# patngnw/NewsRecommendation

Measured on AMD Instinct MI355X. Metric: train impressions/sec @ batch 512, NRMS, higher is better.
Workload: dtype bf16; 1 GPU; NRMS train step (fwd+bwd+Adam), MIND-small shapes: title_len=30, history=50, npratio=4, 300-d word table; per_gpu_batch=512, global_batch=512, vocab_rows=30000, freeze_embedding=False, compact_history=False, dense_batch=False, feed=resident, deterministic=False, optimizer=flat bucket + HIP fused Adam, parallelism=dp1

## Files before the change

newsrecommendation_amd/csrc/nr_api.hip:

```cpp
#include <stdarg.h>
#include <stdio.h>
#include <stdlib.h>
#include <string.h>

#include "nr_gemm.h"

int nr_launch_attn(bool bwd, int dtype, const void* qkv, const float* mask, void* y, const void* dy, void* dqkv, int n, int L,
                   int heads, int d_head, const DropCfg& drop, hipStream_t stream, const uint32_t* tmask = nullptr,
                   const float* bias = nullptr, const int32_t* seq_list = nullptr, const int32_t* seq_count = nullptr,
                   const int32_t* needed = nullptr);
bool nr_attn_pad_ok(int dtype, int L, int d_head, const void* p0, const void* p1);
bool nr_attn_rowsub_ok(int dtype, int L, int d_head, int heads);
bool nr_attn_compact_ok(int dtype, int L, int d_head, int heads);
int nr_launch_attn_bwd_compact(const void* qkv, const float* mask, const void* dy, void* dqkv, int n, int L, int heads, int d_head,
                               const DropCfg& drop, hipStream_t stream, const uint32_t* tmask, const float* bias, const int32_t* seq_list,
                               const int32_t* seq_count, const int32_t* pos, void* dump, float* db, const int32_t* nzf);
int nr_launch_attn_gather_fwd(const void* proj_table, const int32_t* ids, const float* mask, void* y, int n, int L, int heads,
                              int d_head, const DropCfg& drop, hipStream_t stream);
int nr_launch_pool_core_fwd(int dtype, const void* x, const void* e, const float* w2, const float* b2, const float* mask,
                            float* alpha, float* out, int ld_out, int n, int L, int N, int q, hipStream_t s,
                            const int32_t* needed = nullptr);
int nr_launch_pool_core_bwd(int dtype, const void* x, const void* e, const float* w2, const float* alpha, const float* g,
                            int ld_g, void* dpre, float* partial, float* dw2, float* db2, int n, int L, int N, int q,
                            hipStream_t s, const int32_t* seq_nz = nullptr);
// ... 963 lines not shown
  return nr_launch_pool_core_fwd(d->dtype, d->x, e, d->w2, d->b2, d->mask, alpha, out, ld_out, d->n, d->L, d->N, d->q, s, d->seq_needed);
}

int nr_additive_pool_bwd(const nr_pool_desc* d, const void* e, const float* alpha, const float* g, int ld_g, const void* w1_t,
                         int ldw1t, void* dpre, float* partial, float* dw1, float* db1, float* dw2, float* db2, void* dx,
                         nr_stream_t stream) {
  int rc = pool_check(d);
  if (rc) return rc;
  if (d->n == 0) return NR_OK;
  NR_CHECK_ARG(e && alpha && g && dpre && partial && dw1 && db1 && dw2 && db2, "additive_pool_bwd: null operand");
  NR_DEVICE_GUARD(stream, dpre);
  NR_CHECK_ARG(d->partial_bytes >= pool_ws_elems(d->n, d->L, d->q, d->N, d->dtype) * sizeof(float),
               "additive_pool_bwd: partial holds %zu bytes, nr_pool_workspace_bytes() asks for %zu", d->partial_bytes,
               pool_ws_elems(d->n, d->L, d->q, d->N, d->dtype) * sizeof(float));
  float* tn_scratch = partial + pool_ws_ints(d->n, d->L, d->q);
  const size_t tn_floats = pool_tn_floats(d->n, d->L, d->q, d->N, d->dtype);
  hipStream_t s = (hipStream_t)stream;
  const int M = d->n * d->L;
  DetScope det(s);
  det.add(dw1, (size_t)d->q * d->N);
  det.add(db1, (size_t)d->q);
  det.add(dw2, (size_t)d->q);
  det.add(db2, 1);
  if ((rc = det.begin(true, true))) return rc;
  int32_t* ws = nullptr;
  if (pool_has_flags(d)) {
    ws = reinterpret_cast<int32_t*>(partial + pool_ws_used(d->n, d->q));
    if ((rc = nr_launch_row_flags_f32(g, ld_g, d->N, d->n, ws, s))) return rc;
  }
  const int32_t* zero_flags = ws != nullptr ? ws : d->seq_needed;
  if (ws != nullptr && dx != nullptr && w1_t != nullptr && !det.on() && nr_pool_fused_bwd_ok(d->dtype, d->n, d->L, d->N, d->q, ldw1t) && ld_g % 4 == 0 &&
      ((((uintptr_t)d->x) | ((uintptr_t)e) | ((uintptr_t)w1_t) | ((uintptr_t)dpre) | ((uintptr_t)dx) | ((uintptr_t)g)) & 15) == 0 && d->N % 8 == 0) {
    int rows = 0;
    if ((rc = nr_launch_pool_fused_bwd(d->x, d->N, e, d->q, alpha, g, ld_g, d->w2, w1_t, ldw1t, dpre, d->q, dx, d->N, partial,
                                       nr_pool_partial_rows(d->n), ws, d->n, d->L, d->N, d->q, s, &rows, d->dx_far_unwritten)))
      return rc;
    if ((rc = nr_launch_colsum_split(partial, rows, d->q + 1, d->q + 1, dw2, d->q, db2, s))) return rc;
    if ((rc = nr_launch_live_slabs(ws, d->n, d->L, s))) return rc;
    return gemm_tn_live_slabs(ws, d->n, dpre, d->q, d->x, d->N, dw1, d->N, db1, M, d->q, d->N, d->q, d->N, s, 0, tn_scratch, tn_floats);
  }
  if ((rc = nr_launch_pool_core_bwd(d->dtype, d->x, e, d->w2, alpha, g, ld_g, dpre, partial, dw2, db2, d->n, d->L, d->N, d->q, s, zero_flags)))
    return rc;
  RowSrc X = dense_rows(d->x, d->N, d->N);
  if (ws != nullptr) {
    if ((rc = nr_launch_live_slabs(ws, d->n, d->L, s))) return rc;
    if ((rc = gemm_tn_live_slabs(ws, d->n, dpre, d->q, d->x, d->N, dw1, d->N, db1, M, d->q, d->N, d->q, d->N, s, 0, tn_scratch, tn_floats))) return rc;
  } else if ((rc = nr_launch_gemm_tn(d->dtype, dpre, d->q, X, dw1, d->N, db1, M, d->q, d->N, d->q, d->N, s))) {
    return rc;
  }
  if (dx != nullptr) {
    NR_CHECK_ARG(w1_t != nullptr && ldw1t >= d->q, "additive_pool_bwd: w1_t [N, >=q] needed for dx");
    RowSrc P = dense_rows(dpre, d->q, d->q);
    EpiArgs ep = store_epi(dx, d->N, d->dtype, nullptr, 0);
    ep.rowscale = alpha; ep.G = g; ep.ldg = ld_g; ep.L = d->L;
    ep.seq_nz = zero_flags;
    rc = nr_launch_gemm_nt(d->dtype, P, w1_t, ldw1t, M, d->N, d->q, EPI_POOLBWD, ep, s);
  }
  return rc;
}

static int linear_rows(const nr_linear_desc* d, RowSrc* out) {
  NR_CHECK_ARG(d != nullptr, "linear: null descriptor");
  NR_CHECK_ARG(dtype_ok(d->dtype), "linear: bad dtype %d", d->dtype);
  const int ch = nr_chunk(d->dtype);
  NR_CHECK_ARG(d->M >= 0 && d->K >= 1 && d->N >= 1, "linear: bad shape M=%d K=%d N=%d", d->M, d->K, d->N);
  NR_CHECK_ARG(d->ldx >= round_up(d->K, ch) && d->ldw >= round_up(d->K, ch), "linear: ldx=%d / ldw=%d must cover K=%d rounded up to %d",
               d->ldx, d->ldw, d->K, ch);
  NR_CHECK_ARG(d->M == 0 || (d->x && d->w), "linear: null operand");
  RowSrc s = dense_rows(d->x, d->ldx, d->K);
  if (d->src_kind == NR_SRC_GATHER) {
    NR_CHECK_ARG(d->ids != nullptr && d->ids_stride >= 1, "linear: gather source without ids");
// ... 54 lines not shown
```

newsrecommendation_amd/csrc/nr_attn_mfma.hip:

```cpp
#include <stdlib.h>
#include <type_traits>

#include "nr_common.h"

namespace {

constexpr int AW = 4;

template <typename T> struct AT;
template <> struct AT<bf16_t> { static constexpr int SW = 40; };
template <> struct AT<float> { static constexpr int SW = 36; };

struct AttnMArgs {
  const void* qkv;
  const float* mask;
  void* y;
  const void* dy;
  void* dqkv;
  int n, L, heads, d, N;
  int vec;
  float scale;
  DropCfg drop;
  const int32_t* seq_list;
  const int32_t* seq_count;
// ... 1057 lines not shown
          const bf16_t* src = img0 + re * ops + pc.q4(t);
          *reinterpret_cast<bf16x4*>(base + off) = *reinterpret_cast<const bf16x4*>(src);
          *reinterpret_cast<bf16x4*>(base + off + N) = *reinterpret_cast<const bf16x4*>(src + 32 * ops);
          *reinterpret_cast<bf16x4*>(base + off + 2 * N) = *reinterpret_cast<const bf16x4*>(src + 64 * ops);
        }
      } else if (FULL) {
        panel_store_all<PT>(img0, ops, op, N3, pc);
        panel_store_all<PT>(img0 + 32 * ops, ops, op + N, N3, pc);
        panel_store_all<PT>(img0 + 64 * ops, ops, op + 2 * N, N3, pc);
      } else {
        panel_store<PT>(img0, ops, op, N3, pc, hcount);
        panel_store<PT>(img0 + 32 * ops, ops, op + N, N3, pc, hcount);
        panel_store<PT>(img0 + 64 * ops, ops, op + 2 * N, N3, pc, hcount);
      }
    } else {
      bf16_t* op = dqkv + row0 * N3 + (active ? head : 0) * d;
      acc_t_to_global<false>(dq, op, N3, Ls, d, lane, nodrop, 0, 0);
      acc_t_to_global<false>(dk, op + N, N3, Ls, d, lane, nodrop, 0, 0);
      acc_t_to_global<false>(dv, op + 2 * N, N3, Ls, d, lane, nodrop, 0, 0);
    }
    __syncthreads();
    put(pf);
    __syncthreads();
  }
  if (CPT) {
    for (int i = tid; i < hgroups * AW * 3 * DBS; i += AW * 64) {
      const int c = i % DBS, mat = (i / DBS) % 3, head = i / (3 * DBS);
      if (c < d && head < heads) atomicAdd(a.db + mat * N + head * d + c, sDb[i]);
    }
  }
}


__device__ __forceinline__ int clampL(int L, int rb) { return min(32, max(0, L - 32 * rb)); }

template <bool GATHER, int LC = 0, int DC = 0, int HC = 0>
__global__ __launch_bounds__(AW * 64) __attribute__((amdgpu_waves_per_eu(2, 2))) void fwd64_kernel(AttnMArgs a) {
  extern __shared__ __attribute__((aligned(16))) char smem[];
  const int lane = threadIdx.x & 63, wid = __builtin_amdgcn_readfirstlane(threadIdx.x >> 6);
  bf16_t* base = reinterpret_cast<bf16_t*>(smem) + (size_t)wid * 7 * IMG;
  bf16_t *sQ = base, *sK = base + 2 * IMG, *sV = base + 4 * IMG, *sO = base + 6 * IMG;
  float* sMask = reinterpret_cast<float*>(reinterpret_cast<bf16_t*>(smem) + (size_t)AW * 7 * IMG) + wid * 64;
  const bf16_t* qkv = reinterpret_cast<const bf16_t*>(a.qkv);
  bf16_t* y = reinterpret_cast<bf16_t*>(a.y);
  const int L = LC ? LC : a.L, d = DC ? DC : a.d, heads = HC ? HC : a.heads, N = heads * d, h2 = lane >> 5;
  DropCfg nodrop;
  nodrop.key = 0; nodrop.thresh = 0; nodrop.scale = 1.f;
  const int hgroups = (heads + AW - 1) / AW;
  Slice t[2][3];
  int idr[2] = {0, 0};
  int sh_n = 0, ln_n = L, sh_c = 0, ln_c = L;
  bool gen_n = false, gen_c = false;
  auto load_ids = [&](long sb) {
    if (GATHER) {
      const size_t row0 = (size_t)sb * L;
      sh_n = 0; ln_n = L; gen_n = false;
      if (a.mask != nullptr) {
        const float mv = lane < L ? a.mask[row0 + lane] : 0.f;
        const unsigned long long bal = __ballot(mv != 0.f);
        if (bal == 0) {
          sh_n = L; ln_n = 0;
        } else {
          const int s0 = __builtin_ctzll(bal), hi = 64 - __builtin_clzll(bal);
          if (__popcll(bal) == hi - s0) { sh_n = s0; ln_n = hi - s0; } else gen_n = true;
        }
      }
// ... 26 lines not shown
#pragma unroll
        for (int w = 0; w < 3; ++w) slice_load(t[rb][w], src + (size_t)32 * rb * 3 * N + w * N, 3 * N, Lr, d, lane);
      }
    }
  };
  long sb = blockIdx.x;
  if (sb >= a.n) return;
  load_ids(sb);
  load(sb, 0);
  for (; sb < a.n; sb += gridDim.x)
    for (int hgi = 0; hgi < hgroups; ++hgi) {
      const int hraw = hgi * AW + wid;
      const bool active = hraw < heads;
      if (GATHER && hgi == 0) { sh_c = sh_n; ln_c = ln_n; gen_c = gen_n; }
      const int Lc = GATHER ? ln_c : L;
      const bool two = Lc > 32;
      const int head = active ? hraw : 0, Lw = active ? Lc : 0;
      const size_t row0 = (size_t)sb * L;
#pragma unroll
      for (int rb = 0; rb < 2; ++rb) {
        const int Lr = clampL(Lw, rb);
        slice_put<false>(t[rb][0], Lr, d, sQ + rb * IMG, lane, nodrop, 0, 0);
        slice_put<false>(t[rb][1], Lr, d, sK + rb * IMG, lane, nodrop, 0, 0);
        slice_put<false>(t[rb][2], Lr, d, sV + rb * IMG, lane, nodrop, 0, 0);
      }
      sMask[lane] = (lane < Lw) ? ((a.mask && (!GATHER || gen_c)) ? a.mask[row0 + lane] : 1.f) : 0.f;
      if (GATHER && Lc < L) {
        const int hcols = min(AW, heads - hgi * AW) * d, ppr = hcols >> 2, nz = (L - Lc) * ppr;
        for (int u = threadIdx.x; u < nz; u += AW * 64) {
          const int i = u / ppr, c = (u - i * ppr) * 4, row = i < sh_c ? i : i + Lc;
          *reinterpret_cast<bf16x4*>(y + (row0 + row) * N + hgi * AW * d + c) = (bf16x4){(bf16_t)0.f, (bf16_t)0.f, (bf16_t)0.f, (bf16_t)0.f};
        }
      }
      __syncthreads();
      float mk0[16], mk1[16];
#pragma unroll
      for (int r = 0; r < 16; ++r) { mk0[r] = sMask[rowof(r, h2)]; mk1[r] = sMask[32 + rowof(r, h2)]; }
      if (hgi + 1 < hgroups) {
        load(sb, hgi + 1);
      } else if (sb + gridDim.x < a.n) {
        load_ids(sb + gridDim.x);
        load(sb + gridDim.x, 0);
      }
#pragma unroll 1
      for (int qb = 0; qb < (two ? 2 : 1); ++qb) {
        f32x16 s0, s1;
#pragma unroll
        for (int r = 0; r < 16; ++r) { s0[r] = 0.f; s1[r] = 0.f; }
        mm_rr(s0, sK, sQ + qb * IMG, lane);
        if (two) mm_rr(s1, sK + IMG, sQ + qb * IMG, lane);
        const float c2 = a.scale * 1.44269504088896341f;
        float mr = -INFINITY;
#pragma unroll
        for (int r = 0; r < 16; ++r) {
          mr = fmaxf(mr, s0[r]);
          if (GATHER ? two : (32 + rowof(r, h2) < L)) mr = fmaxf(mr, s1[r]);
        }
        mr = fmaxf(mr, __shfl_xor(mr, 32, 64));
        const float m = mr * a.scale, mc = -mr * c2;
        float sum = 0.f;
#pragma unroll
        for (int r = 0; r < 16; ++r) {
          const float e0 = __builtin_amdgcn_exp2f(fmaf(s0[r], c2, mc)) * mk0[r];
          s0[r] = e0;
          sum += e0;
        }
        if (two) {
#pragma unroll
          for (int r = 0; r < 16; ++r) {
            const float e1 = __builtin_amdgcn_exp2f(fmaf(s1[r], c2, mc)) * mk1[r];
            s1[r] = e1;
            sum += e1;
          }
        }
        sum += __shfl_xor(sum, 32, 64);
        const float inv = 1.f / (sum + 1e-8f * __expf(-m));
#pragma unroll
        for (int r = 0; r < 16; ++r) { s0[r] *= inv; s1[r] *= inv; }
        f32x16 ctx;
#pragma unroll
        for (int r = 0; r < 16; ++r) ctx[r] = 0.f;
        mm_xt(ctx, s0, sV, lane);
        if (two) mm_xt(ctx, s1, sV + IMG, lane);
        __syncthreads();
        acc_to_img_t(ctx, 1.f, sO, lane);
        __syncthreads();
        const size_t r0 = row0 + (GATHER ? sh_c : 0) + 32 * qb;
        img_t_to_global<true>(sO, y + r0 * N + head * d, N, clampL(Lw, qb), d, lane, a.drop, (uint32_t)(r0 * N + head * d), (uint32_t)N);
      }
      __syncthreads();
    }
}

template <int LC = 0, int DC = 0, int HC = 0>
__global__ __launch_bounds__(AW * 64) __attribute__((amdgpu_waves_per_eu(2, 2))) void bwd64_kernel(AttnMArgs a) {
  extern __shared__ __attribute__((aligned(16))) char smem[];
  const int lane = threadIdx.x & 63, wid = __builtin_amdgcn_readfirstlane(threadIdx.x >> 6);
  bf16_t* base = reinterpret_cast<bf16_t*>(smem) + (size_t)wid * 9 * IMG;
  bf16_t *sQ = base, *sK = base + 2 * IMG, *sV = base + 4 * IMG, *sG = base + 6 * IMG, *sO = base + 8 * IMG;
  float* sF = reinterpret_cast<float*>(reinterpret_cast<bf16_t*>(smem) + (size_t)AW * 9 * IMG) + wid * 256;
  float *sMask = sF, *sM = sF + 64, *sInv = sF + 128, *sRd = sF + 192;
  const bf16_t* qkv = reinterpret_cast<const bf16_t*>(a.qkv);
  const bf16_t* dy = reinterpret_cast<const bf16_t*>(a.dy);
  bf16_t* dqkv = reinterpret_cast<bf16_t*>(a.dqkv);
  const int L = LC ? LC : a.L, d = DC ? DC : a.d, heads = HC ? HC : a.heads, N = heads * d, h2 = lane >> 5, li = lane & 31;
  DropCfg nodrop;
  nodrop.key = 0; nodrop.thresh = 0; nodrop.scale = 1.f;
  const int hgroups = (heads + AW - 1) / AW;
  for (long sb = blockIdx.x; sb < a.n; sb += gridDim.x)
    for (int hgi = 0; hgi < hgroups; ++hgi) {
      const int hraw = hgi * AW + wid;
      const bool active = hraw < heads;
      const int head = active ? hraw : 0, Lw = active ? L : 0;
      const size_t row0 = (size_t)sb * L;
      const bf16_t* src = qkv + row0 * 3 * N + head * d;
      Slice t[2][4];
#pragma unroll
      for (int rb = 0; rb < 2; ++rb) {
        const int Lr = clampL(Lw, rb);
        const size_t ro = (size_t)32 * rb;
#pragma unroll
        for (int w = 0; w < 3; ++w) slice_load(t[rb][w], src + ro * 3 * N + w * N, 3 * N, Lr, d, lane);
        slice_load(t[rb][3], dy + (row0 + ro) * N + head * d, N, Lr, d, lane);
      }
#pragma unroll
      for (int rb = 0; rb < 2; ++rb) {
        const int Lr = clampL(Lw, rb);
        const size_t ro = (size_t)32 * rb;
        slice_put<false>(t[rb][0], Lr, d, sQ + rb * IMG, lane, nodrop, 0, 0);
        slice_put<false>(t[rb][1], Lr, d, sK + rb * IMG, lane, nodrop, 0, 0);
        slice_put<false>(t[rb][2], Lr, d, sV + rb * IMG, lane, nodrop, 0, 0);
        slice_put<true>(t[rb][3], Lr, d, sG + rb * IMG, lane, a.drop, (uint32_t)((row0 + ro) * N + head * d), (uint32_t)N);
      }
      sMask[lane] = (lane < Lw) ? (a.mask ? a.mask[row0 + lane] : 1.f) : 0.f;
      __syncthreads();
      bf16_t* op = dqkv + row0 * 3 * N + head * d;
#pragma unroll 1
      for (int qb = 0; qb < 2; ++qb) {
        f32x16 s0, s1, p0, p1;
#pragma unroll
        for (int r = 0; r < 16; ++r) { s0[r] = 0.f; s1[r] = 0.f; p0[r] = 0.f; p1[r] = 0.f; }
        mm_rr(s0, sK, sQ + qb * IMG, lane);
        mm_rr(s1, sK + IMG, sQ + qb * IMG, lane);
        mm_rr(p0, sV, sG + qb * IMG, lane);
        mm_rr(p1, sV + IMG, sG + qb * IMG, lane);
        float m = -INFINITY;
#pragma unroll
        for (int r = 0; r < 16; ++r) {
          s0[r] *= a.scale; s1[r] *= a.scale;
          if (rowof(r, h2) < L) m = fmaxf(m, s0[r]);
          if (32 + rowof(r, h2) < L) m = fmaxf(m, s1[r]);
        }
        m = fmaxf(m, __shfl_xor(m, 32, 64));
        float sum = 0.f, rdu = 0.f;
#pragma unroll
        for (int r = 0; r < 16; ++r) {
          const int j = rowof(r, h2);
          const float e0 = (j < L) ? __expf(s0[r] - m) * sMask[j] : 0.f;
          const float e1 = (32 + j < L) ? __expf(s1[r] - m) * sMask[32 + j] : 0.f;
          s0[r] = e0; s1[r] = e1;
          sum += e0 + e1;
          rdu = fmaf(e0, p0[r], fmaf(e1, p1[r], rdu));
        }
        sum += __shfl_xor(sum, 32, 64);
        rdu += __shfl_xor(rdu, 32, 64);
        const float inv = 1.f / (sum + 1e-8f * __expf(-m));
        const float rd = rdu * inv;
#pragma unroll
        for (int r = 0; r < 16; ++r) {
          s0[r] = s0[r] * inv * (p0[r] - rd);
          s1[r] = s1[r] * inv * (p1[r] - rd);
        }
        if (lane < 32) {
          sM[32 * qb + lane] = m;
          sInv[32 * qb + lane] = inv;
          sRd[32 * qb + lane] = rd;
        }
        f32x16 dq;
#pragma unroll
        for (int r = 0; r < 16; ++r) dq[r] = 0.f;
        mm_xt(dq, s0, sK, lane);
        mm_xt(dq, s1, sK + IMG, lane);
        __syncthreads();
        acc_to_img_t(dq, a.scale, sO, lane);
        __syncthreads();
        img_t_to_global<false>(sO, op + (size_t)32 * qb * 3 * N, 3 * N, clampL(Lw, qb), d, lane, nodrop, 0, 0);
      }
      __syncthreads();
#pragma unroll 1
      for (int kb = 0; kb < 2; ++kb) {
        f32x16 dk, dv;
#pragma unroll
        for (int r = 0; r < 16; ++r) { dk[r] = 0.f; dv[r] = 0.f; }
        const float mj = sMask[32 * kb + li];
#pragma unroll
        for (int qb = 0; qb < 2; ++qb) {
          f32x16 s, dp;
#pragma unroll
          for (int r = 0; r < 16; ++r) { s[r] = 0.f; dp[r] = 0.f; }
          mm_rr(s, sQ + qb * IMG, sK + kb * IMG, lane);
          mm_rr(dp, sG + qb * IMG, sV + kb * IMG, lane);
#pragma unroll
          for (int r = 0; r < 16; ++r) {
            const int i = 32 * qb + rowof(r, h2);
            const float pij = __expf(s[r] * a.scale - sM[i]) * mj * sInv[i];
            s[r] = pij;
            dp[r] = pij * (dp[r] - sRd[i]);
          }
          mm_xt(dk, dp, sQ + qb * IMG, lane);
          mm_xt(dv, s, sG + qb * IMG, lane);
        }
        const int Lk = clampL(Lw, kb);
        __syncthreads();
        acc_to_img_t(dk, a.scale, sO, lane);
        __syncthreads();
        img_t_to_global<false>(sO, op + (size_t)32 * kb * 3 * N + N, 3 * N, Lk, d, lane, nodrop, 0, 0);
        __syncthreads();
        acc_to_img_t(dv, 1.f, sO, lane);
        __syncthreads();
        img_t_to_global<false>(sO, op + (size_t)32 * kb * 3 * N + 2 * N, 3 * N, Lk, d, lane, nodrop, 0, 0);
      }
      __syncthreads();
    }
}


template <int RB>
__global__ __launch_bounds__(AW * 64) void fwd_long_kernel(AttnMArgs a) {
  extern __shared__ __attribute__((aligned(16))) char smem[];
  constexpr int NI = 3 * RB + 1;
  const int lane = threadIdx.x & 63, wid = __builtin_amdgcn_readfirstlane(threadIdx.x >> 6);
  bf16_t* base = reinterpret_cast<bf16_t*>(smem) + (size_t)wid * NI * IMG;
  bf16_t *sQ = base, *sK = base + RB * IMG, *sV = base + 2 * RB * IMG, *sO = base + 3 * RB * IMG;
  float* sMask = reinterpret_cast<float*>(reinterpret_cast<bf16_t*>(smem) + (size_t)AW * NI * IMG) + wid * 128;
  const bf16_t* qkv = reinterpret_cast<const bf16_t*>(a.qkv);
  bf16_t* y = reinterpret_cast<bf16_t*>(a.y);
  const int L = a.L, d = a.d, heads = a.heads, N = heads * d, h2 = lane >> 5;
  DropCfg nodrop;
  nodrop.key = 0; nodrop.thresh = 0; nodrop.scale = 1.f;
  const int hgroups = (heads + AW - 1) / AW;
  const float c2 = a.scale * LOG2E;
  for (long sb = blockIdx.x; sb < a.n; sb += gridDim.x)
    for (int hgi = 0; hgi < hgroups; ++hgi) {
      const int hraw = hgi * AW + wid;
      const bool active = hraw < heads;
      const int head = active ? hraw : 0, Lw = active ? L : 0;
      const size_t row0 = (size_t)sb * L;
      const bf16_t* src = qkv + row0 * 3 * N + head * d;
#pragma unroll
      for (int rb = 0; rb < RB; ++rb) {
        const int Lr = clampL(Lw, rb);
        Slice t[3];
#pragma unroll
        for (int w = 0; w < 3; ++w) slice_load(t[w], src + (size_t)32 * rb * 3 * N + w * N, 3 * N, Lr, d, lane);
        slice_put<false>(t[0], Lr, d, sQ + rb * IMG, lane, nodrop, 0, 0);
// ... 591 lines not shown
```

newsrecommendation_amd/csrc/nr_gemm.h:

```cpp
#pragma once
#include "nr_common.h"

enum { ROWS_DENSE = 0, ROWS_GATHER = 1, ROWS_IM2COL3 = 2 };

struct RowSrc {
  const void* base;
  const int32_t* ids;
  int ld;
  int ids_stride;
  int kind;
  int Tlen;
  int Dtrue;
  DropCfg drop;
  int gap;
};

enum {
  EPI_STORE = 0,
  EPI_POOLBWD = 1,
  EPI_SCATTER = 2,
  EPI_STORE_TANH = 3,
};

struct EpiArgs {
// ... 7 lines not shown
  int ldg, L;
  const int32_t* ids;
  int ids_stride;
  int Dtrue;
  DropCfg drop;
  const int32_t* row_count;
  const int32_t* row_idx;
  const int32_t* row_ids;
  const int32_t* seq_nz;
  void* rows_out;
  int ld_rows_out;
  int a_gap;
  const int32_t* a_idx;
  int a_dense;
  int tail_cus;
};

int nr_launch_gemm_nt(int dtype, const RowSrc& A, const void* B, int ldb, int M, int N, int K, int epi,
                      const EpiArgs& ep, hipStream_t stream);
int nr_launch_conv_rows(int dtype, const RowSrc& A, void* out, int n, hipStream_t stream, const int32_t* needed = nullptr, int margin = 0);
int nr_launch_rows_materialize(int dtype, const RowSrc& A, void* out, int ldo, int M, int K, hipStream_t stream,
                               const int32_t* needed = nullptr, int margin = 0, int L = 0, const int32_t* keep_all = nullptr);
int nr_launch_compact_rows(const int32_t* ids, int ids_stride, int M, int32_t* ws, hipStream_t stream);
int nr_launch_sort_rows_by_id(const int32_t* count, const int32_t* rows, const int32_t* ids, int Mmax, int table_rows, int32_t* hist,
                              int32_t* rows_out, int32_t* ids_out, hipStream_t stream, int32_t* k_out = nullptr,
                              int32_t* counted_cursor = nullptr);
int nr_launch_compact_rows_fwd(const int32_t* ids, int M, int n, int L, const void* table_row0, int cols, int32_t* ws,
                               hipStream_t stream, int32_t* posmap = nullptr, int32_t* zero4 = nullptr, int32_t* zhist = nullptr,
                               int nhist = 0);
int nr_launch_bias_rows(void* C, int ldc, int N, const float* bias, const int32_t* rows, const int32_t* count, int max_rows,
                        const uint32_t* tmask, int L, hipStream_t stream);
int nr_launch_title_flags(const void* dy, int n, int L, int N, int32_t* title_nz, hipStream_t stream);
int nr_launch_row_flags_f32(const float* g, int ld, int N, int n, int32_t* nz, hipStream_t stream);
int nr_launch_live_slabs(int32_t* ws, int n, int L, hipStream_t stream);
int nr_launch_needed_list(const int32_t* flags, int n, int32_t* out, void* y, size_t seq_bytes, hipStream_t stream, int reach = -1,
                          bool zeroed = false);
int nr_launch_seq_list(const int32_t* title_nz, const uint32_t* tmask, int n, int L, int32_t* out, hipStream_t stream, int reach = -1,
                       bool zeroed = false);
int nr_launch_zero_tail_rows(void* buf, int ld, const int32_t* count, int Mmax, hipStream_t stream, int32_t* za = nullptr, int na = 0,
                             int32_t* zb = nullptr, int nb = 0);
int nr_launch_gemm_tn_slabs(const void* dC, int ldc, const void* X, int ldx, float* dW, int ldw, float* db, int M, int N, int K,
                            int Nstore, int Kstore, const int32_t* slab_list, const int32_t* slab_count, hipStream_t stream, int xgap = 0,
                            float* scratch = nullptr, size_t scratch_floats = 0);
size_t nr_gemm_tn_scratch_floats(int M, int N, int K);
bool nr_gemm_tn_slabs_ok(int ldc, int ldx, int M, int N, int K);
int nr_pool_fused_fwd_ok(int dtype, int n, int L, int N, int q, int ldw1);
int nr_launch_pool_fused_fwd(const void* x, int ldx, const void* w1, int ldw1, const float* b1, const float* w2, const float* b2,
                             const float* mask, void* e, int lde, float* alpha, float* out, int ld_out, int n, int L, int N, int q,
                             const int32_t* needed, hipStream_t stream);
int nr_launch_gemm_tn_counted(const void* dC, int ldc, const void* X, int ldx, float* dW, int ldw, int Mmax, int N, int K, int Nstore,
                              int Kstore, const int32_t* row_count, hipStream_t stream, float* scratch = nullptr, size_t scratch_floats = 0);
int nr_pool_fused_bwd_ok(int dtype, int n, int L, int N, int q, int ldw1t);
int nr_launch_pool_fused_bwd(const void* x, int ldx, const void* e, int lde, const float* alpha, const float* g, int ldg, const float* w2,
                             const void* w1t, int ldw1t, void* dpre, int ldp, void* dx, int lddx, float* partial, int partial_rows,
                             const int32_t* nz, int n, int L, int N, int q, hipStream_t stream, int* grid_out, int dx_far_unwritten = 0);
int nr_launch_gather_live_rows(int dtype, const RowSrc& A, void* out, int ldo, int Mmax, int K, const int32_t* count, const int32_t* rows,
                               const int32_t* ids, hipStream_t stream, int32_t* hist = nullptr, int V = 0);
int nr_launch_gemm_tn(int dtype, const void* dC, int ldc, const RowSrc& A, float* dW, int ldw, float* db,
                      int M, int N, int K, int Nstore, int Kstore, hipStream_t stream);
int nr_launch_conv_table_live(const int32_t* ids, int ids_stride, const int32_t* seq_nz, int n, int T, int V, int32_t* hdr, int32_t* live_s,
                              int32_t* live_id, hipStream_t stream);
int nr_launch_conv_table_stage(int dtype, const void* dy, int n, int T, int N, const int32_t* hdr, const int32_t* live_s, bool compact, void* out,
                               int32_t* ident, hipStream_t stream);
int nr_launch_conv_table_rank(const int32_t* hdr, const int32_t* sort_s, const int32_t* sort_id, const int32_t* sort_k, const int32_t* cursor,
                              bool compact, int n, int32_t* ord_s, int32_t* ord_slot, hipStream_t stream);
int nr_launch_conv_table_scatter(int dx_dtype, const void* dx, int ldx, int n, int T, int D, int V, const int32_t* hdr, const int32_t* sort_id,
                                 const int32_t* cursor, const int32_t* ord_s, const int32_t* ord_slot, DropCfg drop, float* dtable,
                                 hipStream_t stream);
```

newsrecommendation_amd/csrc/nr_gemm.hip:

```cpp
#include <stdlib.h>

#include "nr_gemm.h"
#include "nr_scatter_tail.h"

namespace {

constexpr int BM = 128, BN = 128, BK = 32, NTHR = 256;
constexpr int SC = BN + 4;

template <typename T> struct TileCfg {
  static constexpr int CH = 16 / (int)sizeof(T);
  static constexpr int SK = BK + CH;
  static constexpr int CPR = BK / CH;
  static constexpr int NCH = BM * CPR / NTHR;
  static constexpr int RPC = BM / CH;
  static constexpr size_t STAGE_BYTES = (size_t)2 * 2 * BM * SK * sizeof(T);
};
constexpr size_t EPI_BYTES = (size_t)64 * SC * sizeof(float);

template <typename T> constexpr size_t smem_bytes() {
  return TileCfg<T>::STAGE_BYTES > EPI_BYTES ? TileCfg<T>::STAGE_BYTES : EPI_BYTES;
}

union Chunk {
// ... 1882 lines not shown
  };

#pragma unroll 1
  for (int k = 0; k < nsteps + 2; ++k) {
    if (k >= 2) asm volatile("s_waitcnt vmcnt(%0)" ::"n"(Cfg::STEADY) : "memory");
    else wait_vmcnt_le(k == 0 ? (NS - 3) * PW : PW + (Cfg::S + 2));
    __builtin_amdgcn_s_barrier();
    issue_stage(k + NS - 2);
    if (wid < NW / 2) {
      phase_gemm(k);
      phase_out(k);
      phase_alpha(k);
    } else {
      phase_out(k);
      phase_alpha(k);
      phase_gemm(k);
    }
  }
}

struct PoolFusedBwdArgs {
  const bf16_t* x; int ldx;
  const bf16_t* e; int lde;
  const float* alpha;
  const float* g; int ldg;
  const float* w2;
  const bf16_t* w1t; int ldw1t;
  bf16_t* dpre; int ldp;
  bf16_t* dx; int lddx;
  float* partial;
  const int32_t* nz;
  int n, L, N, q;
  int dx_far_unwritten;
};

template <int KS, int KS2>
struct PoolFusedBwdCfg {
  static constexpr int NW = 8, TPW = 4, RT = 2, R = 32;
  static constexpr int EPIECES = RT * KS2, GPIECES = 2, PIECES = EPIECES + GPIECES;
  static constexpr int PW = (PIECES + NW - 1) / NW, STAGE = PIECES * 1024, NS = 5;
  static constexpr int LOADS = 5;
  static constexpr int OPS = PW + LOADS + 2 + RT * 2;
  static constexpr int STEADY = 2 * OPS - PW;
  static constexpr int DUMP = NS * STAGE;
  static constexpr int PARTA = DUMP + NW * 1024;
  static constexpr int ALPHA = PARTA + 2 * NW * 32 * 4;
  static constexpr int W2 = ALPHA + 4 * 32 * 4;
  static constexpr int ACCW = W2 + 2 * 256 * 4;
  static constexpr int LIST = ACCW + 512 * 16 * 4;
  static_assert(STEADY <= 62, "vmcnt is a 6-bit counter");
};

template <int KS, int KS2>
__global__ __launch_bounds__(512) void pool_fused_bwd_kernel(PoolFusedBwdArgs a, int reach) {
  using Cfg = PoolFusedBwdCfg<KS, KS2>;
  constexpr int NW = Cfg::NW, TPW = Cfg::TPW, RT = Cfg::RT, NS = Cfg::NS, PW = Cfg::PW, STAGE = Cfg::STAGE, EPIECES = Cfg::EPIECES;
  extern __shared__ __attribute__((aligned(16))) char smem[];
  const uint32_t lds0 = (uint32_t)(size_t)(__attribute__((address_space(3))) char*)smem;
  const int tid = threadIdx.x, lane = tid & 63;
  const int wid = __builtin_amdgcn_readfirstlane(tid >> 6);
  const int fr = lane & 15, g = lane >> 4;
  const int prow = lane >> 2, c8 = ((lane & 3) ^ swzP(prow)) * 8;
  const int L = a.L, N = a.N, q = a.q, M = a.n * a.L, qc = q >> 3;
  float* sPartA = reinterpret_cast<float*>(smem + Cfg::PARTA);
  float* sAlpha = reinterpret_cast<float*>(smem + Cfg::ALPHA);
  float* sW2 = reinterpret_cast<float*>(smem + Cfg::W2);
  float* sRedW = sW2 + 256;
  int* sList = reinterpret_cast<int*>(smem + Cfg::LIST);

  const int G = gridDim.x, b0 = blockIdx.x;
  int nsteps = b0 < a.n ? (a.n - b0 + G - 1) / G : 0;
  if (a.nz != nullptr) {
    __shared__ int sCnt[NW + 1];
    const int cand = nsteps;
    const int run = pool_balanced_walk<NW>(a.nz, a.n, G, b0, sList, sCnt, wid, lane);
    for (int c = wid; c < cand; c += NW) {
      const int sq = b0 + c * G;
      if (a.nz[sq] != 0) continue;
      bool near = false;
      for (int t = max(0, sq - reach) + lane; t <= min(a.n - 1, sq + reach); t += 64) near |= a.nz[t] != 0;
      near = __ballot(near) != 0ull;
      const size_t r0 = (size_t)sq * L;
      const int xc = N >> 3;
      if (near || !a.dx_far_unwritten)
        for (int u = lane; u < L * xc; u += 64) {
          const int row = u / xc, ch = u - row * xc;
          *reinterpret_cast<uint4*>(a.dx + (r0 + row) * a.lddx + ch * 8) = make_uint4(0, 0, 0, 0);
        }
      if (near)
        for (int u = lane; u < L * qc; u += 64) {
          const int row = u / qc, ch = u - row * qc;
          *reinterpret_cast<uint4*>(a.dpre + (r0 + row) * a.ldp + ch * 8) = make_uint4(0, 0, 0, 0);
        }
    }
    nsteps = run;
  } else {
    for (int c = tid; c < nsteps; c += 512) sList[c] = b0 + c * G;
  }
  for (int c = tid; c < 256; c += 512) {
    sW2[c] = c < q ? a.w2[c] : 0.f;
    sRedW[c] = 0.f;
  }
  const int wcol0 = wid * TPW * 16;
  bf16x8 bfr[TPW][KS2];
#pragma unroll
  for (int t = 0; t < TPW; ++t) {
    const bf16_t* brow = a.w1t + (size_t)min(wcol0 + t * 16 + fr, N - 1) * a.ldw1t + 8 * g;
#pragma unroll
    for (int s2 = 0; s2 < KS2; ++s2) bfr[t][s2] = *reinterpret_cast<const bf16x8*>(brow + 32 * s2);
  }
  __builtin_amdgcn_s_waitcnt(0x0F70);
  __syncthreads();
  float* prow_out = a.partial + (size_t)blockIdx.x * (q + 1);
  if (nsteps == 0) {
    for (int c = tid; c <= q; c += 512) prow_out[c] = 0.f;
    return;
  }

  const uint32_t dump_lds = lds0 + Cfg::DUMP + wid * 1024;
  uint4* dump_g = g_nt_dump + wid * 64 + lane;
  auto issue_stage = [&](int kk) {
    const uint32_t slot = lds0 + (kk % NS) * STAGE;
    const bool real = kk < nsteps;
    const int sq = real ? sList[kk] : 0;
    const int row0 = sq * L;
#pragma unroll
    for (int u = 0; u < PW; ++u) {
      const int p = wid + NW * u;
// ... 1113 lines not shown
  using Cfg = PoolFusedCfg<KS>;
  NR_CHECK_ARG(nr_pool_fused_fwd_ok(NR_BF16, n, L, N, q, ldw1) && ldx >= N && ldx % 8 == 0 && lde >= q && lde % 8 == 0 &&
                   ((((uintptr_t)x) | ((uintptr_t)w1) | ((uintptr_t)e)) & 15) == 0 && mask == nullptr,
               "pool_fused_fwd: shape / alignment not eligible (and no mask on this path)");
  static int cus = 0;
  if (cus == 0) {
    int dev = 0, c = 0;
    NR_CHECK_HIP(hipGetDevice(&dev));
    NR_CHECK_HIP(hipDeviceGetAttribute(&c, hipDeviceAttributeMultiprocessorCount, dev));
    cus = c >= 8 ? c : 256;
  }
  const int grid = n < cus ? n : cus;
  const int max_steps = (n + grid - 1) / grid;
  const size_t smem = (size_t)Cfg::LIST + (size_t)(max_steps + 8) * sizeof(int);
  NR_CHECK_ARG(smem <= 160 * 1024, "pool_fused_fwd: %d sequences per workgroup do not fit the LDS list", max_steps);
  PoolFusedArgs a;
  a.x = (const bf16_t*)x; a.ldx = ldx; a.w1 = (const bf16_t*)w1; a.ldw1 = ldw1; a.b1 = b1; a.w2 = w2; a.b2 = b2;
  a.e = (bf16_t*)e; a.lde = lde; a.alpha = alpha; a.out = out; a.ld_out = ld_out; a.needed = needed; a.n = n; a.L = L; a.N = N; a.q = q;
  auto kern = pool_fused_fwd_kernel<KS>;
  NR_CHECK_HIP(hipFuncSetAttribute(reinterpret_cast<const void*>(kern), hipFuncAttributeMaxDynamicSharedMemorySize, (int)smem));
  NrProfScope ps(stream, needed ? "pool_fused_fwd_needed[bf16,n=%d,L=%d,N=%d,q=%d]" : "pool_fused_fwd[bf16,n=%d,L=%d,N=%d,q=%d]", n, L, N, q);
  hipLaunchKernelGGL(kern, dim3(grid), dim3(512), smem, stream, a, max_steps);
  NR_CHECK_LAUNCH();
  return NR_OK;
}

int nr_pool_fused_bwd_ok(int dtype, int n, int L, int N, int q, int ldw1t) {
  return !nr_opt(NR_OPT_NO_POOL_FUSED) && dtype == NR_BF16 && L >= 24 && L <= 32 && N > 384 && N <= 416 && N % 8 == 0 && q > 192 && q <= 224 &&
         q % 8 == 0 && ldw1t >= 224 && (long)n * L >= 4096;
}

int nr_launch_pool_fused_bwd(const void* x, int ldx, const void* e, int lde, const float* alpha, const float* g, int ldg, const float* w2,
                             const void* w1t, int ldw1t, void* dpre, int ldp, void* dx, int lddx, float* partial, int partial_rows,
                             const int32_t* nz, int n, int L, int N, int q, hipStream_t stream, int* grid_out, int dx_far_unwritten) {
  constexpr int KS = 13, KS2 = 7;
  using Cfg = PoolFusedBwdCfg<KS, KS2>;
  NR_CHECK_ARG(nr_pool_fused_bwd_ok(NR_BF16, n, L, N, q, ldw1t) && ldx >= N && ldx % 8 == 0 && lde >= q && lde % 8 == 0 && ldp >= q && ldp % 8 == 0 &&
                   lddx >= N && lddx % 8 == 0 && ldg >= N && ldg % 4 == 0 &&
                   ((((uintptr_t)x) | ((uintptr_t)e) | ((uintptr_t)w1t) | ((uintptr_t)dpre) | ((uintptr_t)dx) | ((uintptr_t)g)) & 15) == 0,
               "pool_fused_bwd: shape / alignment not eligible");
  static int cus = 0;
  if (cus == 0) {
    int dev = 0, c = 0;
    NR_CHECK_HIP(hipGetDevice(&dev));
    NR_CHECK_HIP(hipDeviceGetAttribute(&c, hipDeviceAttributeMultiprocessorCount, dev));
    cus = c >= 8 ? c : 256;
  }
  int grid = n < cus ? n : cus;
  if (grid > partial_rows) grid = partial_rows;
  const int max_steps = (n + grid - 1) / grid;
  const size_t smem = (size_t)Cfg::LIST + (size_t)(max_steps + 8) * sizeof(int);
  NR_CHECK_ARG(smem <= 160 * 1024, "pool_fused_bwd: %d sequences per workgroup do not fit the LDS list", max_steps);
  PoolFusedBwdArgs a;
  a.x = (const bf16_t*)x; a.ldx = ldx; a.e = (const bf16_t*)e; a.lde = lde; a.alpha = alpha; a.g = g; a.ldg = ldg; a.w2 = w2;
  a.w1t = (const bf16_t*)w1t; a.ldw1t = ldw1t; a.dpre = (bf16_t*)dpre; a.ldp = ldp; a.dx = (bf16_t*)dx; a.lddx = lddx; a.partial = partial;
  a.nz = nz; a.n = n; a.L = L; a.N = N; a.q = q; a.dx_far_unwritten = (nz != nullptr && dx_far_unwritten) ? 1 : 0;
  auto kern = pool_fused_bwd_kernel<KS, KS2>;
  NR_CHECK_HIP(hipFuncSetAttribute(reinterpret_cast<const void*>(kern), hipFuncAttributeMaxDynamicSharedMemorySize, (int)smem));
  NrProfScope ps(stream, "pool_fused_bwd[bf16,n=%d,L=%d,N=%d,q=%d]", n, L, N, q);
  hipLaunchKernelGGL(kern, dim3(grid), dim3(512), smem, stream, a, 32 / L + 2);
  NR_CHECK_LAUNCH();
  *grid_out = grid;
  return NR_OK;
}

int nr_launch_gather_live_rows(int dtype, const RowSrc& A, void* out, int ldo, int Mmax, int K, const int32_t* count, const int32_t* rows,
                               const int32_t* ids, hipStream_t stream, int32_t* hist, int V) {
  const int ch = nr_chunk(dtype);
  NR_CHECK_ARG(A.kind == ROWS_GATHER && K % ch == 0 && ldo % ch == 0 && ldo >= K && A.ld >= K && count && rows && ids && out,
               "gather_live_rows: bad arguments");
  NrProfScope ps(stream, "rows_materialize_live[%s,Mmax=%d,K=%d]", dtype == NR_BF16 ? "bf16" : "f32", Mmax, K);
  const size_t total = (size_t)Mmax * (K / ch);
  size_t grid = (total + 256 * 4 - 1) / (256 * 4);
  if (grid > 256 * 16) grid = 256 * 16;
  if (grid < 1) grid = 1;
  if (dtype == NR_BF16)
    hipLaunchKernelGGL(gather_live_rows_kernel<bf16_t>, dim3((unsigned)grid), dim3(256), 0, stream, A, (bf16_t*)out, ldo, K, count, rows, ids, hist, V);
  else
    hipLaunchKernelGGL(gather_live_rows_kernel<float>, dim3((unsigned)grid), dim3(256), 0, stream, A, (float*)out, ldo, K, count, rows, ids, hist, V);
  NR_CHECK_LAUNCH();
  return NR_OK;
}

int nr_launch_gemm_nt(int dtype, const RowSrc& A, const void* B, int ldb, int M, int N, int K, int epi, const EpiArgs& ep,
                      hipStream_t stream) {
  const int ch = nr_chunk(dtype);
  NR_CHECK_ARG(M > 0 && N > 0 && K > 0, "gemm_nt: empty problem M=%d N=%d K=%d", M, N, K);
  NR_CHECK_ARG(K % ch == 0 && ldb % ch == 0 && A.ld % ch == 0, "gemm_nt: K=%d ldb=%d lda=%d must be multiples of %d", K, ldb, A.ld, ch);
  NR_CHECK_ARG(((uintptr_t)A.base & 15) == 0 && ((uintptr_t)B & 15) == 0, "gemm_nt: operands must be 16-byte aligned");
// ... 293 lines not shown
  NR_CHECK_LAUNCH();
  return NR_OK;
}

int nr_launch_seq_list(const int32_t* title_nz, const uint32_t* tmask, int n, int L, int32_t* out, hipStream_t stream, int reach, bool zeroed) {
  if (!zeroed) NR_CHECK_HIP(hipMemsetAsync(out, 0, 4 * sizeof(int32_t), stream));
  hipLaunchKernelGGL(seq_list_kernel, dim3((n + 255) / 256), dim3(256), 0, stream, title_nz, tmask, n, reach >= 0 ? reach : 32 / L + 2, out,
                     out + 4);
  NR_CHECK_LAUNCH();
  return NR_OK;
}

namespace {
__global__ __launch_bounds__(256) void zero_tail_rows_kernel(uint4* __restrict__ buf, int chunks, const int32_t* __restrict__ count, int Mmax,
                                                             int32_t* __restrict__ za, int na, int32_t* __restrict__ zb, int nb) {
  const int t = blockIdx.x * 256 + threadIdx.x, stride = gridDim.x * 256;
  for (int i = t; i < na; i += stride) za[i] = 0;
  for (int i = t; i < nb; i += stride) zb[i] = 0;
  if (blockIdx.x != 0) return;
  const int n = *count, end = min(Mmax, (n + 31) / 32 * 32);
  for (int u = threadIdx.x; u < (end - n) * chunks; u += 256) buf[(size_t)n * chunks + u] = make_uint4(0, 0, 0, 0);
}
}
int nr_launch_zero_tail_rows(void* buf, int ld, const int32_t* count, int Mmax, hipStream_t stream, int32_t* za, int na, int32_t* zb, int nb) {
  NR_CHECK_ARG(buf != nullptr && count != nullptr && ld % 8 == 0 && (((uintptr_t)buf) & 15) == 0, "zero_tail_rows: bad arguments");
  if (za == nullptr) na = 0;
  if (zb == nullptr) nb = 0;
  const int most = na > nb ? na : nb, grid = most > 4096 ? 16 : 1;
  hipLaunchKernelGGL(zero_tail_rows_kernel, dim3(grid), dim3(256), 0, stream, (uint4*)buf, ld / 8, count, Mmax, za, na, zb, nb);
  NR_CHECK_LAUNCH();
  return NR_OK;
}

int nr_launch_live_slabs(int32_t* ws, int n, int L, hipStream_t stream) {
  const int M = n * L, nslab = M / 32;
  NR_CHECK_ARG(ws != nullptr && M % 32 == 0, "live_slabs: bad arguments");
  int32_t* list = ws + n + 4;
  if (nslab >= 4 && nslab <= 128 * 1024) {
    unsigned char* flags = reinterpret_cast<unsigned char*>(list + nslab - (nslab + 3) / 4);
    hipLaunchKernelGGL(slab_flags_kernel, dim3((nslab + 255) / 256), dim3(256), 0, stream, ws, n, L, nslab, flags);
    hipLaunchKernelGGL(slab_list_kernel, dim3(1), dim3(1024), (size_t)((nslab + 15) / 16) * 16, stream, flags, nslab, ws + n, list);
    NR_CHECK_LAUNCH();
    return NR_OK;
  }
  const int in_lds = n <= 128 * 1024 ? 1 : 0;
  hipLaunchKernelGGL(live_slabs_kernel, dim3(1), dim3(1024), in_lds ? (size_t)((n + 15) / 16) * 16 : 0, stream, ws, n, L, nslab, ws + n,
                     list, in_lds);
  NR_CHECK_LAUNCH();
  return NR_OK;
}

int nr_launch_gemm_tn_slabs(const void* dC, int ldc, const void* X, int ldx, float* dW, int ldw, float* db, int M, int N, int K,
                            int Nstore, int Kstore, const int32_t* slab_list, const int32_t* slab_count, hipStream_t stream, int xgap,
                            float* scratch, size_t scratch_floats) {
  NR_CHECK_ARG(tn3::eligible(ldc, ldx, M, N, K), "gemm_tn_slabs: shape not eligible");
  NrProfScope ps(stream, "gemm_tn3_live[bf16,Mmax=%d,N=%d,K=%d,gap=%d]", M, N, K, xgap);
  return tn3::launch(dC, ldc, X, ldx, dW, ldw, db, M, N, K, Nstore, Kstore, stream, slab_list, slab_count, xgap, scratch, scratch_floats);
}
size_t nr_gemm_tn_scratch_floats(int M, int N, int K) { return tn3::scratch_floats(M, N, K); }
bool nr_gemm_tn_slabs_ok(int ldc, int ldx, int M, int N, int K) { return tn3::eligible(ldc, ldx, M, N, K); }
int nr_launch_gemm_tn_counted(const void* dC, int ldc, const void* X, int ldx, float* dW, int ldw, int Mmax, int N, int K, int Nstore,
                              int Kstore, const int32_t* row_count, hipStream_t stream, float* scratch, size_t scratch_floats) {
  NR_CHECK_ARG(tn3::eligible(ldc, ldx, Mmax, N, K) && row_count != nullptr, "gemm_tn_counted: shape not eligible");
  NrProfScope ps(stream, "gemm_tn3_rows[bf16,Mmax=%d,N=%d,K=%d,gap=0]", Mmax, N, K);
  return tn3::launch(dC, ldc, X, ldx, dW, ldw, nullptr, Mmax, N, K, Nstore, Kstore, stream, nullptr, row_count, 0, scratch, scratch_floats);
}

int nr_launch_gemm_tn(int dtype, const void* dC, int ldc, const RowSrc& A, float* dW, int ldw, float* db, int M, int N,
                      int K, int Nstore, int Kstore, hipStream_t stream) {
  const int ch = nr_chunk(dtype);
  NR_CHECK_ARG(M > 0 && N > 0 && K > 0, "gemm_tn: empty problem M=%d N=%d K=%d", M, N, K);
  NR_CHECK_ARG(N % ch == 0 && K % ch == 0 && ldc % ch == 0 && A.ld % ch == 0, "gemm_tn: N=%d K=%d ldc=%d lda=%d must be multiples of %d",
               N, K, ldc, A.ld, ch);
  NR_CHECK_ARG(((uintptr_t)A.base & 15) == 0 && ((uintptr_t)dC & 15) == 0, "gemm_tn: operands must be 16-byte aligned");
  if (dtype == NR_BF16 && A.kind == ROWS_DENSE && A.drop.thresh == 0) {
    if (tn3::eligible(ldc, A.ld, M, N, K)) {
      NrProfScope ps(stream, "gemm_tn3[bf16,M=%d,N=%d,K=%d,gap=%d]", M, N, K, A.gap);
// ... 12 lines not shown
```

Before: 178,900 impressions/s.

## Replace block barriers with wave-level LDS sync in attention and fold slab flags into pool backward

In the MFMA attention forward and backward kernels, each wave works on its own LDS region, so the block-wide __syncthreads calls are replaced by wavefront-scope fences plus a wave barrier. This lets waves proceed independently and avoids stalls across the whole block. Separately, the fused additive-pool backward kernel now writes the live-slab flag bytes itself, which removes the separate slab_flags kernel launch before slab list construction. The risk is a correctness hazard if any of the LDS data is in fact shared between waves, and a possible race if the flag writes are not ordered before the list kernel reads them.

```diff
diff --git a/newsrecommendation_amd/csrc/nr_api.hip b/newsrecommendation_amd/csrc/nr_api.hip
--- a/newsrecommendation_amd/csrc/nr_api.hip
+++ b/newsrecommendation_amd/csrc/nr_api.hip
@@ -1019,11 +1019,12 @@
   if (ws != nullptr && dx != nullptr && w1_t != nullptr && !det.on() && nr_pool_fused_bwd_ok(d->dtype, d->n, d->L, d->N, d->q, ldw1t) && ld_g % 4 == 0 &&
       ((((uintptr_t)d->x) | ((uintptr_t)e) | ((uintptr_t)w1_t) | ((uintptr_t)dpre) | ((uintptr_t)dx) | ((uintptr_t)g)) & 15) == 0 && d->N % 8 == 0) {
     int rows = 0;
+    unsigned char* slab_flags = nr_live_slab_flags(ws, d->n, d->L);
     if ((rc = nr_launch_pool_fused_bwd(d->x, d->N, e, d->q, alpha, g, ld_g, d->w2, w1_t, ldw1t, dpre, d->q, dx, d->N, partial,
-                                       nr_pool_partial_rows(d->n), ws, d->n, d->L, d->N, d->q, s, &rows, d->dx_far_unwritten)))
+                                       nr_pool_partial_rows(d->n), ws, d->n, d->L, d->N, d->q, s, &rows, d->dx_far_unwritten, slab_flags)))
       return rc;
     if ((rc = nr_launch_colsum_split(partial, rows, d->q + 1, d->q + 1, dw2, d->q, db2, s))) return rc;
-    if ((rc = nr_launch_live_slabs(ws, d->n, d->L, s))) return rc;
+    if ((rc = nr_launch_live_slabs(ws, d->n, d->L, s, slab_flags != nullptr))) return rc;
     return gemm_tn_live_slabs(ws, d->n, dpre, d->q, d->x, d->N, dw1, d->N, db1, M, d->q, d->N, d->q, d->N, s, 0, tn_scratch, tn_floats);
   }
   if ((rc = nr_launch_pool_core_bwd(d->dtype, d->x, e, d->w2, alpha, g, ld_g, dpre, partial, dw2, db2, d->n, d->L, d->N, d->q, s, zero_flags)))
diff --git a/newsrecommendation_amd/csrc/nr_attn_mfma.hip b/newsrecommendation_amd/csrc/nr_attn_mfma.hip
--- a/newsrecommendation_amd/csrc/nr_attn_mfma.hip
+++ b/newsrecommendation_amd/csrc/nr_attn_mfma.hip
@@ -1113,6 +1113,11 @@
 }
 
 
+__device__ __forceinline__ void wave_lds_sync() {
+  __builtin_amdgcn_fence(__ATOMIC_RELEASE, "wavefront");
+  __builtin_amdgcn_wave_barrier();
+  __builtin_amdgcn_fence(__ATOMIC_ACQUIRE, "wavefront");
+}
 __device__ __forceinline__ int clampL(int L, int rb) { return min(32, max(0, L - 32 * rb)); }
 
 template <bool GATHER, int LC = 0, int DC = 0, int HC = 0>
@@ -1205,7 +1210,7 @@
           *reinterpret_cast<bf16x4*>(y + (row0 + row) * N + hgi * AW * d + c) = (bf16x4){(bf16_t)0.f, (bf16_t)0.f, (bf16_t)0.f, (bf16_t)0.f};
         }
       }
-      __syncthreads();
+      wave_lds_sync();
       float mk0[16], mk1[16];
 #pragma unroll
       for (int r = 0; r < 16; ++r) { mk0[r] = sMask[rowof(r, h2)]; mk1[r] = sMask[32 + rowof(r, h2)]; }
@@ -1255,13 +1260,13 @@
         for (int r = 0; r < 16; ++r) ctx[r] = 0.f;
         mm_xt(ctx, s0, sV, lane);
         if (two) mm_xt(ctx, s1, sV + IMG, lane);
-        __syncthreads();
+        wave_lds_sync();
         acc_to_img_t(ctx, 1.f, sO, lane);
-        __syncthreads();
+        wave_lds_sync();
         const size_t r0 = row0 + (GATHER ? sh_c : 0) + 32 * qb;
         img_t_to_global<true>(sO, y + r0 * N + head * d, N, clampL(Lw, qb), d, lane, a.drop, (uint32_t)(r0 * N + head * d), (uint32_t)N);
       }
-      __syncthreads();
+      wave_lds_sync();
     }
 }
 
@@ -1306,7 +1311,7 @@
         slice_put<true>(t[rb][3], Lr, d, sG + rb * IMG, lane, a.drop, (uint32_t)((row0 + ro) * N + head * d), (uint32_t)N);
       }
       sMask[lane] = (lane < Lw) ? (a.mask ? a.mask[row0 + lane] : 1.f) : 0.f;
-      __syncthreads();
+      wave_lds_sync();
       bf16_t* op = dqkv + row0 * 3 * N + head * d;
 #pragma unroll 1
       for (int qb = 0; qb < 2; ++qb) {
@@ -1354,12 +1359,12 @@
         for (int r = 0; r < 16; ++r) dq[r] = 0.f;
         mm_xt(dq, s0, sK, lane);
         mm_xt(dq, s1, sK + IMG, lane);
-        __syncthreads();
+        wave_lds_sync();
         acc_to_img_t(dq, a.scale, sO, lane);
-        __syncthreads();
+        wave_lds_sync();
         img_t_to_global<false>(sO, op + (size_t)32 * qb * 3 * N, 3 * N, clampL(Lw, qb), d, lane, nodrop, 0, 0);
       }
-      __syncthreads();
+      wave_lds_sync();
 #pragma unroll 1
       for (int kb = 0; kb < 2; ++kb) {
         f32x16 dk, dv;
@@ -1384,16 +1389,16 @@
           mm_xt(dv, s, sG + qb * IMG, lane);
         }
         const int Lk = clampL(Lw, kb);
-        __syncthreads();
+        wave_lds_sync();
         acc_to_img_t(dk, a.scale, sO, lane);
-        __syncthreads();
+        wave_lds_sync();
         img_t_to_global<false>(sO, op + (size_t)32 * kb * 3 * N + N, 3 * N, Lk, d, lane, nodrop, 0, 0);
-        __syncthreads();
+        wave_lds_sync();
         acc_to_img_t(dv, 1.f, sO, lane);
-        __syncthreads();
+        wave_lds_sync();
         img_t_to_global<false>(sO, op + (size_t)32 * kb * 3 * N + 2 * N, 3 * N, Lk, d, lane, nodrop, 0, 0);
       }
-      __syncthreads();
+      wave_lds_sync();
     }
 }
 
diff --git a/newsrecommendation_amd/csrc/nr_gemm.h b/newsrecommendation_amd/csrc/nr_gemm.h
--- a/newsrecommendation_amd/csrc/nr_gemm.h
+++ b/newsrecommendation_amd/csrc/nr_gemm.h
@@ -63,7 +63,8 @@
                         const uint32_t* tmask, int L, hipStream_t stream);
 int nr_launch_title_flags(const void* dy, int n, int L, int N, int32_t* title_nz, hipStream_t stream);
 int nr_launch_row_flags_f32(const float* g, int ld, int N, int n, int32_t* nz, hipStream_t stream);
-int nr_launch_live_slabs(int32_t* ws, int n, int L, hipStream_t stream);
+int nr_launch_live_slabs(int32_t* ws, int n, int L, hipStream_t stream, bool flags_ready = false);
+unsigned char* nr_live_slab_flags(int32_t* ws, int n, int L);
 int nr_launch_needed_list(const int32_t* flags, int n, int32_t* out, void* y, size_t seq_bytes, hipStream_t stream, int reach = -1,
                           bool zeroed = false);
 int nr_launch_seq_list(const int32_t* title_nz, const uint32_t* tmask, int n, int L, int32_t* out, hipStream_t stream, int reach = -1,
@@ -84,7 +85,8 @@
 int nr_pool_fused_bwd_ok(int dtype, int n, int L, int N, int q, int ldw1t);
 int nr_launch_pool_fused_bwd(const void* x, int ldx, const void* e, int lde, const float* alpha, const float* g, int ldg, const float* w2,
                              const void* w1t, int ldw1t, void* dpre, int ldp, void* dx, int lddx, float* partial, int partial_rows,
-                             const int32_t* nz, int n, int L, int N, int q, hipStream_t stream, int* grid_out, int dx_far_unwritten = 0);
+                             const int32_t* nz, int n, int L, int N, int q, hipStream_t stream, int* grid_out, int dx_far_unwritten = 0,
+                             unsigned char* slab_flags = nullptr);
 int nr_launch_gather_live_rows(int dtype, const RowSrc& A, void* out, int ldo, int Mmax, int K, const int32_t* count, const int32_t* rows,
                                const int32_t* ids, hipStream_t stream, int32_t* hist = nullptr, int V = 0);
 int nr_launch_gemm_tn(int dtype, const void* dC, int ldc, const RowSrc& A, float* dW, int ldw, float* db,
diff --git a/newsrecommendation_amd/csrc/nr_gemm.hip b/newsrecommendation_amd/csrc/nr_gemm.hip
--- a/newsrecommendation_amd/csrc/nr_gemm.hip
+++ b/newsrecommendation_amd/csrc/nr_gemm.hip
@@ -1938,6 +1938,8 @@
   const int32_t* nz;
   int n, L, N, q;
   int dx_far_unwritten;
+  unsigned char* slab_flags;
+  int nslab;
 };
 
 template <int KS, int KS2>
@@ -2000,6 +2002,13 @@
         }
     }
     nsteps = run;
+    if (a.slab_flags != nullptr)
+      for (int s = b0 * 512 + tid; s < a.nslab; s += G * 512) {
+        const int t0 = (32 * s) / L, t1 = min(a.n - 1, (32 * s + 31) / L);
+        bool lv = false;
+        for (int t = t0; t <= t1; ++t) lv |= a.nz[t] != 0;
+        a.slab_flags[s] = lv ? 1 : 0;
+      }
   } else {
     for (int c = tid; c < nsteps; c += 512) sList[c] = b0 + c * G;
   }
@@ -3179,7 +3188,8 @@
 
 int nr_launch_pool_fused_bwd(const void* x, int ldx, const void* e, int lde, const float* alpha, const float* g, int ldg, const float* w2,
                              const void* w1t, int ldw1t, void* dpre, int ldp, void* dx, int lddx, float* partial, int partial_rows,
-                             const int32_t* nz, int n, int L, int N, int q, hipStream_t stream, int* grid_out, int dx_far_unwritten) {
+                             const int32_t* nz, int n, int L, int N, int q, hipStream_t stream, int* grid_out, int dx_far_unwritten,
+                             unsigned char* slab_flags) {
   constexpr int KS = 13, KS2 = 7;
   using Cfg = PoolFusedBwdCfg<KS, KS2>;
   NR_CHECK_ARG(nr_pool_fused_bwd_ok(NR_BF16, n, L, N, q, ldw1t) && ldx >= N && ldx % 8 == 0 && lde >= q && lde % 8 == 0 && ldp >= q && ldp % 8 == 0 &&
@@ -3202,6 +3212,7 @@
   a.x = (const bf16_t*)x; a.ldx = ldx; a.e = (const bf16_t*)e; a.lde = lde; a.alpha = alpha; a.g = g; a.ldg = ldg; a.w2 = w2;
   a.w1t = (const bf16_t*)w1t; a.ldw1t = ldw1t; a.dpre = (bf16_t*)dpre; a.ldp = ldp; a.dx = (bf16_t*)dx; a.lddx = lddx; a.partial = partial;
   a.nz = nz; a.n = n; a.L = L; a.N = N; a.q = q; a.dx_far_unwritten = (nz != nullptr && dx_far_unwritten) ? 1 : 0;
+  a.slab_flags = nz != nullptr ? slab_flags : nullptr; a.nslab = n * L / 32;
   auto kern = pool_fused_bwd_kernel<KS, KS2>;
   NR_CHECK_HIP(hipFuncSetAttribute(reinterpret_cast<const void*>(kern), hipFuncAttributeMaxDynamicSharedMemorySize, (int)smem));
   NrProfScope ps(stream, "pool_fused_bwd[bf16,n=%d,L=%d,N=%d,q=%d]", n, L, N, q);
@@ -3561,17 +3572,22 @@
   return NR_OK;
 }
 
-int nr_launch_live_slabs(int32_t* ws, int n, int L, hipStream_t stream) {
+unsigned char* nr_live_slab_flags(int32_t* ws, int n, int L) {
+  const int nslab = n * L / 32;
+  if (ws == nullptr || (n * L) % 32 != 0 || nslab < 4 || nslab > 128 * 1024) return nullptr;
+  return reinterpret_cast<unsigned char*>(ws + n + 4 + nslab - (nslab + 3) / 4);
+}
+int nr_launch_live_slabs(int32_t* ws, int n, int L, hipStream_t stream, bool flags_ready) {
   const int M = n * L, nslab = M / 32;
   NR_CHECK_ARG(ws != nullptr && M % 32 == 0, "live_slabs: bad arguments");
   int32_t* list = ws + n + 4;
-  if (nslab >= 4 && nslab <= 128 * 1024) {
-    unsigned char* flags = reinterpret_cast<unsigned char*>(list + nslab - (nslab + 3) / 4);
-    hipLaunchKernelGGL(slab_flags_kernel, dim3((nslab + 255) / 256), dim3(256), 0, stream, ws, n, L, nslab, flags);
+  if (unsigned char* flags = nr_live_slab_flags(ws, n, L)) {
+    if (!flags_ready) hipLaunchKernelGGL(slab_flags_kernel, dim3((nslab + 255) / 256), dim3(256), 0, stream, ws, n, L, nslab, flags);
     hipLaunchKernelGGL(slab_list_kernel, dim3(1), dim3(1024), (size_t)((nslab + 15) / 16) * 16, stream, flags, nslab, ws + n, list);
     NR_CHECK_LAUNCH();
     return NR_OK;
   }
+  NR_CHECK_ARG(!flags_ready, "live_slabs: no flag bytes at this size (nr_live_slab_flags)");
   const int in_lds = n <= 128 * 1024 ? 1 : 0;
   hipLaunchKernelGGL(live_slabs_kernel, dim3(1), dim3(1024), in_lds ? (size_t)((n + 15) / 16) * 16 : 0, stream, ws, n, L, nslab, ws + n,
                      list, in_lds);
```

Measured after the change: 178,900 impressions/s, median of 2. About the same (-0.0%).
